# POSTECH-CVLab/RoDyGS

Measured on AMD Instinct MI355X. Metric: train-step fps at 1M dynamic Gaussians / 1080p (fwd+bwd+Adam, one camera per GPU per step), higher is better.
Workload: dtype f32; 1 GPU; 1000000 dynamic Gaussians + deformation MLP, 1920x1080, SH3, 100-frame synthetic video (BASELINE configs[2]); points=1000000, width=1920, height=1080, scene=uniform, frames=100, deferred_overflow_check=True, frame_order=orbit positions, bit-reversed, one_device=False, graph_replay=False, densify_stats=True, deterministic_backward=True, render_normal=True, parallelism=single GPU (frame-dp1), losses=photometric, sh_adam_in_backward=True, binning=bucket

## Files before the change

### rodygs_amd/csrc/rdg_common.h

```cpp
#pragma once
#include <hip/hip_runtime.h>
#include <stdint.h>
#include <stddef.h>
#include "../../include/rodygs_hip.h"

#define RDG_TILE 16
#define RDG_TILE_PIX 256
#define RDG_WAVE 64

#define RDG_NEAR_CULL 0.2f
#define RDG_FOV_CLAMP 1.3f
#define RDG_DILATION 0.3f
#define RDG_ALPHA_CAP 0.99f
#define RDG_ALPHA_MIN (1.0f / 255.0f)
#define RDG_T_STOP 0.0001f
#define RDG_LAMBDA_FLOOR 0.1f

struct __attribute__((aligned(64))) RdgRec {
    float4 q0, q1, q2, q3;
};

#define RDG_GROW 16

static inline size_t rdg_align_up(size_t x, size_t a) { return (x + a - 1) / a * a; }
// ... 230 lines not shown
                              const float* grow, float* posebuf, float* dmeans3D, float* dmeans2D, float* dshs,
                              float* dcolors, float* dopac, float* dscales, float* drots, float* dcov3D,
                              float* dview, hipStream_t s, const RdgShAdam* sh_adam = nullptr);

int rdg_launch_preprocess_fwd_views(const RdgDev& d, int32_t nviews, int32_t stride, int32_t row0,
                                    const float* means3D, const float* shs, const float* opac, const float* scales,
                                    const float* rots, const float* views, const float* proj, void* geom_ws,
                                    int32_t* radii, hipStream_t s);
int rdg_launch_preprocess_bwd_views(const RdgDev& d, int32_t nviews, int32_t stride, const float* means3D,
                                    const float* shs, const float* opac, const float* scales, const float* rots,
                                    const float* views, const float* proj, const int32_t* radii, const void* geom_ws,
                                    const float* grow, float* posebuf, float* dmeans3D, float* dmeans2D, float* dshs,
                                    float* dopac, float* dscales, float* drots, hipStream_t s);
int rdg_launch_pose_reduce_views(int nviews, int view_rows, int nblk, const float* views, float* posebuf, float* part,
                                 float* dviews, hipStream_t s);

#ifdef __HIPCC__
template <int CTRL, int ROW_MASK = 0xf, int BANK_MASK = 0xf, bool BOUND = true>
__device__ __forceinline__ float rdg_dpp(float x) {
    return __builtin_bit_cast(float, __builtin_amdgcn_update_dpp(0, __builtin_bit_cast(int, x), CTRL, ROW_MASK,
                                                                 BANK_MASK, BOUND));
}
template <int CTRL, int ROW_MASK = 0xf, int BANK_MASK = 0xf, bool BOUND = true>
__device__ __forceinline__ uint32_t rdg_dpp_u(uint32_t x) {
    return (uint32_t)__builtin_amdgcn_update_dpp(0, (int)x, CTRL, ROW_MASK, BANK_MASK, BOUND);
}
__device__ __forceinline__ float rdg_wave_sum_to63(float x) {
    x += rdg_dpp<0xB1>(x);
    x += rdg_dpp<0x4E>(x);
    x += rdg_dpp<0x141>(x);
    x += rdg_dpp<0x140>(x);
    x += rdg_dpp<0x142, 0xa>(x);
    x += rdg_dpp<0x143, 0xc>(x);
    return x;
}
__device__ __forceinline__ float rdg_wave_sum_all(float x) {
    x = rdg_wave_sum_to63(x);
    return __builtin_bit_cast(float, __builtin_amdgcn_readlane(__builtin_bit_cast(int, x), 63));
}
__device__ __forceinline__ void rdg_wave_lds_sync() {
    __builtin_amdgcn_fence(__ATOMIC_RELEASE, "wavefront");
    __builtin_amdgcn_wave_barrier();
    __builtin_amdgcn_fence(__ATOMIC_ACQUIRE, "wavefront");
}

template <bool NT = true>
__device__ __forceinline__ void rdg_rows_to_lds(const float* __restrict__ g, long long first_row, long long n_rows,
                                                int row, int stride, float* S, int lane) {
    const long long base = first_row * row, total = n_rows * row;
    const float inv_row = 1.0f / (float)row;
    if ((row & 3) == 0 && (((uintptr_t)g) & 15) == 0) {
        typedef float rdg_nt4 __attribute__((ext_vector_type(4)));
        for (int v0 = lane; v0 < 16 * row; v0 += 256) {
            rdg_nt4 val[4];
#pragma unroll
            for (int u = 0; u < 4; ++u) {
                const int v = v0 + 64 * u;
                const long long e = base + 4ll * v;
                if (v < 16 * row && e < total)
                    val[u] = NT ? __builtin_nontemporal_load(reinterpret_cast<const rdg_nt4*>(g + e))
                                : *reinterpret_cast<const rdg_nt4*>(g + e);
            }
#pragma unroll
            for (int u = 0; u < 4; ++u) {
                const int v = v0 + 64 * u;
                const long long e = base + 4ll * v;
                if (v < 16 * row && e < total) {
                    const int gi = (int)(((float)(4 * v) + 0.5f) * inv_row);
                    float* dst = S + gi * stride + (4 * v - gi * row);
                    dst[0] = val[u].x; dst[1] = val[u].y; dst[2] = val[u].z; dst[3] = val[u].w;
                }
            }
        }
    } else {
        for (int idx = lane; idx < 64 * row; idx += 64) {
            const long long e = base + idx;
            if (e < total) {
                const int gi = (int)(((float)idx + 0.5f) * inv_row);
                S[gi * stride + (idx - gi * row)] = g[e];
            }
        }
    }
}
__device__ __forceinline__ void rdg_lds_to_rows(float* __restrict__ g, long long first_row, long long n_rows, int row,
                                                int stride, const float* S, int lane) {
    const long long base = first_row * row, total = n_rows * row;
    const float inv_row = 1.0f / (float)row;
    if ((row & 3) == 0 && (((uintptr_t)g) & 15) == 0) {
        for (int v = lane; v < 16 * row; v += 64) {
            const long long e = base + 4ll * v;
            if (e < total) {
                const int gi = (int)(((float)(4 * v) + 0.5f) * inv_row);
                const float* src = S + gi * stride + (4 * v - gi * row);
                typedef float rdg_nt4 __attribute__((ext_vector_type(4)));
                const rdg_nt4 val = {src[0], src[1], src[2], src[3]};
                __builtin_nontemporal_store(val, reinterpret_cast<rdg_nt4*>(g + e));
            }
        }
    } else {
        for (int idx = lane; idx < 64 * row; idx += 64) {
            const long long e = base + idx;
            if (e < total) {
                const int gi = (int)(((float)idx + 0.5f) * inv_row);
                g[e] = S[gi * stride + (idx - gi * row)];
            }
        }
    }
}
template <bool ACC>
__device__ __forceinline__ void rdg_lds_acc_rows(float* __restrict__ g, long long first_row, long long n_rows, int row,
                                                 int stride, const float* S, int lane) {
    const long long base = first_row * row, total = n_rows * row;
    const float inv_row = 1.0f / (float)row;
    if ((row & 3) == 0 && (((uintptr_t)g) & 15) == 0) {
        for (int v = lane; v < 16 * row; v += 64) {
            const long long e = base + 4ll * v;
            if (e < total) {
                const int gi = (int)(((float)(4 * v) + 0.5f) * inv_row);
                const float* src = S + gi * stride + (4 * v - gi * row);
                float4* dst = reinterpret_cast<float4*>(g + e);
                float4 val = make_float4(src[0], src[1], src[2], src[3]);
                if (ACC) { const float4 o = *dst; val.x += o.x; val.y += o.y; val.z += o.z; val.w += o.w; }
                *dst = val;
            }
        }
    } else {
        for (int idx = lane; idx < 64 * row; idx += 64) {
            const long long e = base + idx;
            if (e < total) {
                const int gi = (int)(((float)idx + 0.5f) * inv_row);
                const float val = S[gi * stride + (idx - gi * row)];
                g[e] = ACC ? g[e] + val : val;
            }
        }
    }
}
__device__ __forceinline__ void rdg_adam_elem(float& p, float g, float& m, float& v, float st, float b1, float b2,
                                              float omb1, float omb2, float eps, float bc2_sqrt) {
    m = __fmaf_rn(b1, m, omb1 * g);
    v = __fmaf_rn(b2, v, (omb2 * g) * g);
    p = __fmaf_rn(-st, m / (sqrtf(v) / bc2_sqrt + eps), p);
}


#define RDG_FAC 20
__device__ __forceinline__ float rdg_fac_grad(const float* Frow, int idx) {
    const int k = (idx * 171) >> 9;
    return Frow[k] * Frow[16 + (idx - 3 * k)];
}
__device__ __forceinline__ void rdg_lds_adam_rows_fac(float* __restrict__ p, const RdgShAdam ad, long long first_row,
                                                      long long n_rows, int row, int stride, const float* S,
                                                      const float* F, int lane) {
    const long long base = first_row * row, total = n_rows * row;
    const float inv_row = 1.0f / (float)row;
    typedef float rdg_nt4 __attribute__((ext_vector_type(4)));
    if ((row & 3) == 0 && ((((uintptr_t)p) | ((uintptr_t)ad.m) | ((uintptr_t)ad.v)) & 15) == 0) {
#define RDG_ADAM_UNROLL 4
        for (int v0 = lane; v0 < 16 * row; v0 += 64 * RDG_ADAM_UNROLL) {
            rdg_nt4 mm[RDG_ADAM_UNROLL], vv[RDG_ADAM_UNROLL];
#pragma unroll
            for (int u = 0; u < RDG_ADAM_UNROLL; ++u) {
                const int v = v0 + 64 * u;
                const long long e = base + 4ll * v;
                if (v < 16 * row && e < total) {
                    mm[u] = __builtin_nontemporal_load(reinterpret_cast<const rdg_nt4*>(ad.m + e));
                    vv[u] = __builtin_nontemporal_load(reinterpret_cast<const rdg_nt4*>(ad.v + e));
// ... 90 lines not shown
```

### rodygs_amd/csrc/rdg_preprocess_fwd.hip

```cpp
#include "rdg_common.h"

#define SH_C0 0.28209479177387814f
#define SH_C1 0.4886025119029199f
__device__ static const float SH_C2[5] = {1.0925484305920792f, -1.0925484305920792f, 0.31539156525252005f,
                                          -1.0925484305920792f, 0.5462742152960396f};
__device__ static const float SH_C3[7] = {-0.5900435899266435f, 2.890611442640554f, -0.4570457994644658f,
                                          0.3731763325901154f,  -0.4570457994644658f, 1.445305721320277f,
                                          -0.5900435899266435f};

__device__ __forceinline__ void rdg_rect(float px, float py, int radius, int gx, int gy, int& x0, int& y0,
                                         int& x1, int& y1) {
    float r = (float)radius;
    x0 = min(gx, max(0, (int)((px - r) / (float)RDG_TILE)));
    y0 = min(gy, max(0, (int)((py - r) / (float)RDG_TILE)));
    x1 = min(gx, max(0, (int)((((px + r) + (float)RDG_TILE) - 1.0f) / (float)RDG_TILE)));
    y1 = min(gy, max(0, (int)((((py + r) + (float)RDG_TILE) - 1.0f) / (float)RDG_TILE)));
}

__device__ __forceinline__ float rdg_ln_exact_ops(float x) {
    const uint32_t u = __float_as_uint(x);
    int e = (int)(u >> 23) - 127;
    float m = __uint_as_float((u & 0x007fffffu) | 0x3f800000u);
    if (m > 1.41421354f) { m = m * 0.5f; e += 1; }
    const float s = (m - 1.0f) / (m + 1.0f);
    const float s2 = s * s;
    float p = 0.111111111f * s2 + 0.142857143f;
    p = p * s2 + 0.2f;
    p = p * s2 + 0.333333333f;
    p = p * s2 + 1.0f;
    return (2.0f * s) * p + (float)e * 0.693147181f;
}

__device__ __forceinline__ void rdg_splat_rect(const float4 q0, const float4 q1, const float inv_cyy, int gx, int gy, int cull,
                                               int& x0, int& y0, int& x1, int& y1) {
    rdg_rect(q0.x, q0.y, __float_as_int(q1.w), gx, gy, x0, y0, x1, y1);
    if (!cull) return;
    const float a = q0.z, b = q0.w, o = q1.y;
    const float t255 = 255.0f * o;
    if (!(t255 >= 0.99f)) { x1 = x0; y1 = y0; return; }
    const float r2 = (2.0f * (rdg_ln_exact_ops(t255) + 0.02f)) * 1.001f;
    const float cyy = 1.0f / inv_cyy;
    const float c_eff = (b * b) / a + inv_cyy;
    const float cxx = (c_eff * cyy) / a;
    const float hx = sqrtf(r2 * cxx), hy = sqrtf(r2 * cyy);
    const float lox = fmaxf(ceilf(q0.x - hx), 0.0f), hix = fminf(floorf(q0.x + hx), (float)(gx * RDG_TILE - 1));
    const float loy = fmaxf(ceilf(q0.y - hy), 0.0f), hiy = fminf(floorf(q0.y + hy), (float)(gy * RDG_TILE - 1));
    if (hix < lox || hiy < loy) { x1 = x0; y1 = y0; return; }
    x0 = max(x0, (int)lox >> 4); x1 = min(x1, ((int)hix >> 4) + 1);
    y0 = max(y0, (int)loy >> 4); y1 = min(y1, ((int)hiy >> 4) + 1);
    if (x1 < x0) x1 = x0;
    if (y1 < y0) y1 = y0;
}
__device__ __forceinline__ uint4 rdg_pack_rectd(int x0, int y0, int x1, int y1, float depth, uint32_t tiles) {
    if (tiles == 0u) return make_uint4(0u, 0u, 0u, 0u);
    return make_uint4((uint32_t)x0 | ((uint32_t)y0 << 16), (uint32_t)x1 | ((uint32_t)y1 << 16), __float_as_uint(depth), tiles);
}

template <bool MULTI>
__global__ void __launch_bounds__(RDG_PRE_BLOCK)
rdg_preprocess_fwd_kernel(RdgDev d, const float* __restrict__ view_b, const float* __restrict__ proj,
                          const float* __restrict__ means3D_b, const float* __restrict__ shs,
                          const float* __restrict__ colors, const float* __restrict__ opac,
                          const float* __restrict__ scales, const float* __restrict__ rots_b,
                          const float* __restrict__ cov3Dp, RdgRec* __restrict__ rec_b,
                          uint32_t* __restrict__ tiles_touched_b, uint8_t* __restrict__ clampedm_b,
                          uint32_t* __restrict__ block_sums_b, int32_t* __restrict__ radii_b, int nviews_arg,
                          int vstride_arg, int blk0_arg, uint4* __restrict__ rectd_b) {
    const int nviews = MULTI ? nviews_arg : 1, vstride = MULTI ? vstride_arg : 0;
    const int bid = (MULTI ? blk0_arg : 0) + (int)blockIdx.x;
    const int i = bid * RDG_PRE_BLOCK + threadIdx.x;
    __shared__ float sSH[RDG_PRE_BLOCK / 64][64 * 49];
    const int sh_row = d.M * 3, sh_stride = sh_row | 1;
    const long long wave_first = (long long)bid * RDG_PRE_BLOCK + (threadIdx.x >> 6) * 64;
    if (shs && wave_first < d.P) {
        rdg_rows_to_lds(shs, wave_first, d.P, sh_row, sh_stride, sSH[threadIdx.x >> 6], threadIdx.x & 63);
        rdg_wave_lds_sync();
    }
    __shared__ uint32_t wsum[RDG_PRE_BLOCK / RDG_WAVE];
    for (int vw = 0; vw < nviews; ++vw) {
    const size_t vo = (size_t)vw * vstride;
    const float* __restrict__ view = view_b + 16 * vw;
    const float* __restrict__ means3D = means3D_b + vo * 3;
    const float* __restrict__ rots = rots_b ? rots_b + vo * 4 : nullptr;
    RdgRec* __restrict__ rec = rec_b + vo;
    uint32_t* __restrict__ tiles_touched = tiles_touched_b + vo;
    uint8_t* __restrict__ clampedm = clampedm_b + vo;
    int32_t* __restrict__ radii = radii_b + vo;
    uint32_t* __restrict__ block_sums = block_sums_b + vo / RDG_PRE_BLOCK;
    uint4* __restrict__ rectd = rectd_b + vo;
    float V[16], Pm[16];
#pragma unroll
    for (int k = 0; k < 16; ++k) { V[k] = view[k]; Pm[k] = proj[k]; }
    uint32_t my_tiles = 0;
    if (i < d.P) {
        int radius_out = 0;
        uint8_t cl = 0;
        uint4 rd = make_uint4(0u, 0u, 0u, 0u);
        RdgRec R;
        R.q0 = make_float4(0.f, 0.f, 0.f, 0.f);
        R.q1 = R.q0; R.q2 = R.q0; R.q3 = R.q0;
        const float x = means3D[3 * i + 0], y = means3D[3 * i + 1], z = means3D[3 * i + 2];
        const float vx = ((V[0] * x + V[4] * y) + V[8] * z) + V[12];
        const float vy = ((V[1] * x + V[5] * y) + V[9] * z) + V[13];
        const float vz = ((V[2] * x + V[6] * y) + V[10] * z) + V[14];
        bool valid = vz > RDG_NEAR_CULL;
        if (valid) {
            const float hx = ((Pm[0] * vx + Pm[4] * vy) + Pm[8] * vz) + Pm[12];
            const float hy = ((Pm[1] * vx + Pm[5] * vy) + Pm[9] * vz) + Pm[13];
            const float hw = ((Pm[3] * vx + Pm[7] * vy) + Pm[11] * vz) + Pm[15];
            const float pw = 1.0f / (hw + 1e-7f);
            const float ndc_x = hx * pw, ndc_y = hy * pw;

            float S00, S01, S02, S11, S12, S22;
            float nx = 0.f, ny = 0.f, nz = 0.f;
            if (cov3Dp) {
                S00 = cov3Dp[6 * i + 0]; S01 = cov3Dp[6 * i + 1]; S02 = cov3Dp[6 * i + 2];
                S11 = cov3Dp[6 * i + 3]; S12 = cov3Dp[6 * i + 4]; S22 = cov3Dp[6 * i + 5];
            } else {
                const float s0 = d.smod * scales[3 * i + 0], s1 = d.smod * scales[3 * i + 1],
                            s2 = d.smod * scales[3 * i + 2];
                const float4 q = reinterpret_cast<const float4*>(rots)[i];
                const float r = q.x, qx = q.y, qy = q.z, qz = q.w;
                const float R00 = 1.0f - 2.0f * (qy * qy + qz * qz), R01 = 2.0f * (qx * qy - r * qz),
                            R02 = 2.0f * (qx * qz + r * qy);
                const float R10 = 2.0f * (qx * qy + r * qz), R11 = 1.0f - 2.0f * (qx * qx + qz * qz),
                            R12 = 2.0f * (qy * qz - r * qx);
                const float R20 = 2.0f * (qx * qz - r * qy), R21 = 2.0f * (qy * qz + r * qx),
                            R22 = 1.0f - 2.0f * (qx * qx + qy * qy);
                const float L00 = R00 * s0, L01 = R01 * s1, L02 = R02 * s2;
                const float L10 = R10 * s0, L11 = R11 * s1, L12 = R12 * s2;
                const float L20 = R20 * s0, L21 = R21 * s1, L22 = R22 * s2;
                S00 = (L00 * L00 + L01 * L01) + L02 * L02;
                S01 = (L00 * L10 + L01 * L11) + L02 * L12;
                S02 = (L00 * L20 + L01 * L21) + L02 * L22;
                S11 = (L10 * L10 + L11 * L11) + L12 * L12;
                S12 = (L10 * L20 + L11 * L21) + L12 * L22;
                S22 = (L20 * L20 + L21 * L21) + L22 * L22;
                if (d.render_normal) {
                    const float sc0 = scales[3 * i + 0], sc1 = scales[3 * i + 1], sc2 = scales[3 * i + 2];
                    int k = 0; float sm = sc0;
                    if (sc1 < sm) { sm = sc1; k = 1; }
                    if (sc2 < sm) { sm = sc2; k = 2; }
                    const float n0 = k == 0 ? R00 : (k == 1 ? R01 : R02);
                    const float n1 = k == 0 ? R10 : (k == 1 ? R11 : R12);
                    const float n2 = k == 0 ? R20 : (k == 1 ? R21 : R22);
                    float nvx = (V[0] * n0 + V[4] * n1) + V[8] * n2;
                    float nvy = (V[1] * n0 + V[5] * n1) + V[9] * n2;
                    float nvz = (V[2] * n0 + V[6] * n1) + V[10] * n2;
                    const float dotv = (nvx * vx + nvy * vy) + nvz * vz;
                    const float sg = dotv > 0.f ? -1.0f : 1.0f;
                    nx = nvx * sg; ny = nvy * sg; nz = nvz * sg;
                }
            }
            const float limx = RDG_FOV_CLAMP * d.tanx, limy = RDG_FOV_CLAMP * d.tany;
            const float txtz = vx / vz, tytz = vy / vz;
            const float tx = fminf(limx, fmaxf(-limx, txtz)) * vz;
            const float ty = fminf(limy, fmaxf(-limy, tytz)) * vz;
            const float J00 = d.fx / vz, J02 = -(d.fx * tx) / (vz * vz);
            const float J11 = d.fy / vz, J12 = -(d.fy * ty) / (vz * vz);
            const float T00 = J00 * V[0] + J02 * V[2], T01 = J00 * V[4] + J02 * V[6], T02 = J00 * V[8] + J02 * V[10];
            const float T10 = J11 * V[1] + J12 * V[2], T11 = J11 * V[5] + J12 * V[6], T12 = J11 * V[9] + J12 * V[10];
            const float u00 = (T00 * S00 + T01 * S01) + T02 * S02;
            const float u01 = (T00 * S01 + T01 * S11) + T02 * S12;
            const float u02 = (T00 * S02 + T01 * S12) + T02 * S22;
            const float u10 = (T10 * S00 + T11 * S01) + T12 * S02;
            const float u11 = (T10 * S01 + T11 * S11) + T12 * S12;
            const float u12 = (T10 * S02 + T11 * S12) + T12 * S22;
            const float ca = ((u00 * T00 + u01 * T01) + u02 * T02) + RDG_DILATION;
            const float cb = (u00 * T10 + u01 * T11) + u02 * T12;
            const float cc = ((u10 * T10 + u11 * T11) + u12 * T12) + RDG_DILATION;
            const float det = ca * cc - cb * cb;
            valid = det != 0.0f;
            if (valid) {
                const float det_inv = 1.0f / det;
                const float mid = 0.5f * (ca + cc);
                const float disc = sqrtf(fmaxf(RDG_LAMBDA_FLOOR, mid * mid - det));
                const float lam = fmaxf(mid + disc, mid - disc);
                const int radius = (int)ceilf(3.0f * sqrtf(lam));
                const float px = ((ndc_x + 1.0f) * (float)d.W - 1.0f) * 0.5f;
                const float py = ((ndc_y + 1.0f) * (float)d.H - 1.0f) * 0.5f;
                const float4 rq0 = make_float4(px, py, cc * det_inv, -cb * det_inv);
                const float4 rq1 = make_float4(ca * det_inv, opac[i], vz, __int_as_float(radius));
                const float inv_cyy = 1.0f / cc;
                int x0, y0, x1, y1;
                rdg_rect(px, py, radius, d.gx, d.gy, x0, y0, x1, y1);
                const int area = (x1 - x0) * (y1 - y0);
                if (area > 0) {
                    if (d.cull) rdg_splat_rect(rq0, rq1, inv_cyy, d.gx, d.gy, 1, x0, y0, x1, y1);
                    my_tiles = (uint32_t)((x1 - x0) * (y1 - y0));
                    rd = rdg_pack_rectd(x0, y0, x1, y1, vz, my_tiles);
                    radius_out = radius;
                    float cr, cg, cbl;
                    if (colors) {
                        cr = colors[3 * i + 0]; cg = colors[3 * i + 1]; cbl = colors[3 * i + 2];
                    } else {
                        const float camx = -((V[0] * V[12] + V[1] * V[13]) + V[2] * V[14]);
                        const float camy = -((V[4] * V[12] + V[5] * V[13]) + V[6] * V[14]);
                        const float camz = -((V[8] * V[12] + V[9] * V[13]) + V[10] * V[14]);
                        float dx = x - camx, dy = y - camy, dz = z - camz;
                        const float ln = sqrtf((dx * dx + dy * dy) + dz * dz);
                        dx = dx / ln; dy = dy / ln; dz = dz / ln;
                        const float* sh = sSH[threadIdx.x >> 6] + (threadIdx.x & 63) * sh_stride;
                        float res[3];
#pragma unroll
                        for (int c = 0; c < 3; ++c) res[c] = SH_C0 * sh[c];
                        if (d.deg > 0) {
#pragma unroll
                            for (int c = 0; c < 3; ++c)
                                res[c] = res[c] - SH_C1 * dy * sh[3 + c] + SH_C1 * dz * sh[6 + c] -
                                         SH_C1 * dx * sh[9 + c];
                            if (d.deg > 1) {
                                const float xx = dx * dx, yy = dy * dy, zz = dz * dz;
                                const float xy = dx * dy, yz = dy * dz, xz = dx * dz;
#pragma unroll
                                for (int c = 0; c < 3; ++c)
                                    res[c] = res[c] + SH_C2[0] * xy * sh[12 + c] + SH_C2[1] * yz * sh[15 + c] +
                                             SH_C2[2] * (2.0f * zz - xx - yy) * sh[18 + c] +
                                             SH_C2[3] * xz * sh[21 + c] + SH_C2[4] * (xx - yy) * sh[24 + c];
                                if (d.deg > 2) {
#pragma unroll
                                    for (int c = 0; c < 3; ++c)
                                        res[c] = res[c] + SH_C3[0] * dy * (3.0f * xx - yy) * sh[27 + c] +
                                                 SH_C3[1] * xy * dz * sh[30 + c] +
                                                 SH_C3[2] * dy * (4.0f * zz - xx - yy) * sh[33 + c] +
                                                 SH_C3[3] * dz * (2.0f * zz - 3.0f * xx - 3.0f * yy) * sh[36 + c] +
                                                 SH_C3[4] * dx * (4.0f * zz - xx - yy) * sh[39 + c] +
                                                 SH_C3[5] * dz * (xx - yy) * sh[42 + c] +
                                                 SH_C3[6] * dx * (xx - 3.0f * yy) * sh[45 + c];
                                }
                            }
                        }
                        res[0] += 0.5f; res[1] += 0.5f; res[2] += 0.5f;
                        if (res[0] < 0.f) cl |= 1;
                        if (res[1] < 0.f) cl |= 2;
                        if (res[2] < 0.f) cl |= 4;
                        cr = fmaxf(res[0], 0.f); cg = fmaxf(res[1], 0.f); cbl = fmaxf(res[2], 0.f);
                    }
                    R.q0 = rq0;
                    R.q1 = rq1;
                    R.q2 = make_float4(cr, cg, cbl, inv_cyy);
                    R.q3 = make_float4(nx, ny, nz, 0.f);
                }
            }
        }
        rec[i] = R;
        tiles_touched[i] = my_tiles;
        rectd[i] = rd;
        clampedm[i] = cl;
        radii[i] = radius_out;
    }
    uint32_t inc = rdg_wave_scan_incl(my_tiles);
    const uint32_t lane = threadIdx.x & 63, w = threadIdx.x >> 6;
    if (lane == 63) wsum[w] = inc;
    __syncthreads();
    if (threadIdx.x == 0) block_sums[bid] = wsum[0] + wsum[1] + wsum[2] + wsum[3];
    if (nviews > 1) __syncthreads();
    }
}

__global__ void __launch_bounds__(1024) rdg_scan_block_sums_kernel(uint32_t* __restrict__ block_sums, int nblk,
                                                                   int32_t* __restrict__ num_rendered,
                                                                   uint32_t* __restrict__ zero_buf, int zero_words,
                                                                   int32_t* __restrict__ nren_max) {
    for (int i = threadIdx.x; i < zero_words; i += 1024) zero_buf[i] = 0u;
    __shared__ uint32_t wtot[16];
    __shared__ unsigned long long wtot64[16];
    const uint32_t lane = threadIdx.x & 63, w = threadIdx.x >> 6;
    const int per = (nblk + 1023) / 1024;
    const int t0 = min(nblk, (int)threadIdx.x * per), t1 = min(nblk, t0 + per);
    uint32_t mine = 0;
    unsigned long long mine64 = 0ull;
    for (int c0 = t0; c0 < t1; c0 += 8) {
        uint32_t vv[8];
#pragma unroll
        for (int q = 0; q < 8; ++q) vv[q] = c0 + q < t1 ? block_sums[c0 + q] : 0u;
#pragma unroll
        for (int q = 0; q < 8; ++q) { mine += vv[q]; mine64 += vv[q]; }
// ... 112 lines not shown
```

### rodygs_amd/csrc/rdg_render.hip

```cpp
#include "rdg_common.h"

#define RDG_BATCH 256

__device__ __forceinline__ int rdg_tile_of_block(int bid, int n_tiles) {
    const int per = (n_tiles + 7) >> 3;
    return (bid & 7) * per + (bid >> 3);
}

__device__ __forceinline__ float rdg_edge_min(float a, float b2, float c, float inv_c, float ue, float v0, float v1) {
    const float t = b2 * ue;
    const float vs = __builtin_amdgcn_fmed3f(-0.5f * t * inv_c, v0, v1);
    return fmaf(fmaf(c, vs, t), vs, a * ue * ue);
}
__device__ __forceinline__ uint32_t rdg_quadrant_bits(const float4 q0, const float4 q1, const float inv_cyy, float X0, float Y0) {
    const float a = q0.z, b = q0.w, o = q1.y;
    const float c = (b * b) / a + inv_cyy;
    const float t255 = 255.0f * o;
    if (!(t255 >= 0.99f)) return 0u;
    const float det = a * c - b * b;
    if (!(det > 0.0f) || !(a > 0.0f) || !(c > 0.0f)) return 0u;
    const float r2 = 2.0f * (__logf(t255) + 0.02f) * 1.001f;
    const float inv_a = 1.0f / a, inv_c = 1.0f / c, b2 = 2.0f * b;
    uint32_t bits = 0u;
#pragma unroll
    for (int qy = 0; qy < 2; ++qy) {
        const float v1 = q0.y - (Y0 + 8.0f * qy), v0 = v1 - 7.0f;
#pragma unroll
        for (int qx = 0; qx < 2; ++qx) {
            const float u1 = q0.x - (X0 + 8.0f * qx), u0 = u1 - 7.0f;
            const bool inside = u0 <= 0.0f && u1 >= 0.0f && v0 <= 0.0f && v1 >= 0.0f;
            const float m = fminf(fminf(rdg_edge_min(a, b2, c, inv_c, u0, v0, v1), rdg_edge_min(a, b2, c, inv_c, u1, v0, v1)),
                                  fminf(rdg_edge_min(c, b2, a, inv_a, v0, u0, u1), rdg_edge_min(c, b2, a, inv_a, v1, u0, u1)));
            bits |= (uint32_t)(inside || !(m > r2)) << (qy * 2 + qx);
        }
    }
    return bits;
}

#define RDG_NEG_LOG2E (-1.4426950408889634f)
struct RdgConicS { float hA, beta, gam; };
__device__ __forceinline__ RdgConicS rdg_stage_conic(float a, float b, float inv_cyy) {
    const float A2 = RDG_NEG_LOG2E * a, B = RDG_NEG_LOG2E * b;
    RdgConicS s;
    s.hA = 0.5f * A2;
    s.beta = (A2 < 0.0f) ? B / A2 : 0.0f;
    s.gam = (0.5f * RDG_NEG_LOG2E) * inv_cyy;
    return s;
}
__device__ __forceinline__ float rdg_log2_gauss(float hA, float beta, float gam, float dx, float dy) {
    const float w = fmaf(beta, dy, dx);
    return fmaf(hA * w, w, (gam * dy) * dy);
}
__device__ __forceinline__ float rdg_log2_gauss_w(float hA, float beta, float gam, float dx, float dy, float& w) {
    w = fmaf(beta, dy, dx);
    return fmaf(hA * w, w, (gam * dy) * dy);
}

__device__ __forceinline__ bool rdg_any(bool p) { return __builtin_amdgcn_ballot_w64(p) != 0ull; }
__device__ __forceinline__ bool rdg_all(bool p) { return __builtin_amdgcn_ballot_w64(!p) == 0ull; }

__device__ __forceinline__ unsigned long long rdg_uniform_u64(unsigned long long v) {
    const uint32_t lo = __builtin_amdgcn_readfirstlane((uint32_t)v);
    const uint32_t hi = __builtin_amdgcn_readfirstlane((uint32_t)(v >> 32));
    return ((unsigned long long)hi << 32) | lo;
}

#define RDG_THR_LIVE (0x80000000u | 0x3b808081u)
#define RDG_THR_DONE 0xffffffffu
template <bool NORMAL, bool CAPPED>
__device__ __forceinline__ void rdg_fwd_walk(unsigned long long mask, const unsigned long long cap, const int sbase,
                                             const uint32_t wbase, const char* sQ0, const char* sQ1, const char* sQ2,
                                             const char* sQ3, const float pixx, const float pixy,
                                             unsigned long long& seen, uint32_t& thrU, float& T,
                                             uint32_t& last_contributor, float& C0, float& C1, float& C2, float& Dp,
                                             float& N0, float& N1, float& N2) {
    while (mask) {
        const int jb = __builtin_ctzll(mask);
        asm("s_bitset0_b64 %0, %1" : "+s"(mask) : "s"(jb));
        int aj = (jb << 4) + sbase;
        asm volatile("" : "+v"(aj));
#ifdef RDG_ABL_FXSALU
        asm volatile("s_add_u32 s90, s90, 1\n\ts_add_u32 s91, s91, 1\n\ts_add_u32 s90, s90, 1\n\ts_add_u32 s91, s91, 1\n\t"
                     "s_add_u32 s90, s90, 1\n\ts_add_u32 s91, s91, 1\n\ts_add_u32 s90, s90, 1\n\ts_add_u32 s91, s91, 1" ::: "s90", "s91", "scc");
#endif
#ifdef RDG_ABL_FXVALU
        { float xa = T, xb = C0;
          asm volatile("v_mov_b32 %0, %1\n\tv_mov_b32 %1, %0\n\tv_mov_b32 %0, %1\n\tv_mov_b32 %1, %0\n\t"
                       "v_mov_b32 %0, %1\n\tv_mov_b32 %1, %0\n\tv_mov_b32 %0, %1\n\tv_mov_b32 %1, %0" : "+v"(xa), "+v"(xb)); }
#endif
        const float4 q0 = *(const float4*)(sQ0 + aj);
        const float2 q1 = *(const float2*)(sQ1 + aj);
        const float dx = q0.x - pixx, dy = q0.y - pixy;
        const float power = rdg_log2_gauss(q0.z, q0.w, q1.x, dx, dy);
        float alpha = q1.y * __builtin_amdgcn_exp2f(power);
        if (CAPPED && ((cap >> jb) & 1ull)) {
            asm volatile("; opacity above the cap" ::: "memory");
            alpha = fminf(RDG_ALPHA_CAP, alpha);
        }
        const uint32_t key = (__float_as_uint(power) & 0x80000000u) | __float_as_uint(alpha);
        const unsigned long long cand = __builtin_amdgcn_ballot_w64(key >= thrU);
        if (!cand) continue;
        asm("s_bitset1_b64 %0, %1" : "+s"(seen) : "s"(jb));
        float aeff;
        asm("v_cndmask_b32_e64 %0, 0, %1, %2" : "=v"(aeff) : "v"(alpha), "s"(cand));
        float test_T = T * (1.0f - aeff);
        float wgt = aeff * T;
        const float4 q2 = *(const float4*)(sQ2 + aj);
        const uint32_t idx = wbase + (uint32_t)jb;
        unsigned long long upd = cand;
        const unsigned long long stopm = __builtin_amdgcn_ballot_w64(test_T < RDG_T_STOP);
        if (stopm) {
            const bool stop = test_T < RDG_T_STOP;
            upd &= ~stopm;
            wgt = stop ? 0.0f : wgt;
            test_T = stop ? T : test_T;
            thrU = stop ? RDG_THR_DONE : thrU;
            if (rdg_all(thrU == RDG_THR_DONE)) { mask = 0ull; }
        }
        T = test_T;
        asm volatile("s_mov_b64 exec, %1\n\tv_mov_b32 %0, %2\n\ts_mov_b64 exec, -1"
                     : "+v"(last_contributor) : "s"(upd), "s"(idx));
        C0 += wgt * q2.x; C1 += wgt * q2.y; C2 += wgt * q2.z;
        Dp += wgt * q2.w;
        if (NORMAL) {
            const float4 q3 = *(const float4*)(sQ3 + aj);
            N0 += wgt * q3.x; N1 += wgt * q3.y; N2 += wgt * q3.z;
        }
    }
}


template <bool NORMAL>
__device__ __forceinline__ void
rdg_fwd_composite(const int k_begin, const int k_end, const uint2 range, const float X0, const float Y0, const float pixx,
                  const float pixy, const uint32_t* __restrict__ point_list, const RdgRec* __restrict__ rec,
                  unsigned long long* __restrict__ hit, float4* sQ0, float4* sQ1, float4* sQ2, float4* sQ3,
                  unsigned long long (*sMask)[4], unsigned long long* sCap, uint32_t& thrU, float& T, float& C0, float& C1,
                  float& C2, float& Dp, float& N0, float& N1, float& N2, uint32_t& last_contributor) {
    const int tid = threadIdx.x;
    const int lane = tid & 63, wv = tid >> 6;
    const int rounds = (k_end - k_begin + RDG_BATCH - 1) / RDG_BATCH;
    for (int r = 0; r < rounds; ++r) {
        if (__syncthreads_count(thrU == RDG_THR_DONE) == 256) break;
        const int k = k_begin + r * RDG_BATCH + tid;
        uint32_t qbits = 0;
        bool over_cap = false;
        if (k < k_end) {
            const uint32_t id = point_list[range.x + k];
            const RdgRec* p = rec + id;
            const float4 q0 = p->q0, q1 = p->q1, q2 = p->q2;
            const RdgConicS cs = rdg_stage_conic(q0.z, q0.w, q2.w);
            sQ0[tid] = make_float4(q0.x, q0.y, cs.hA, cs.beta);
            *(float2*)&sQ1[tid] = make_float2(cs.gam, q1.y);
            sQ2[tid] = make_float4(q2.x, q2.y, q2.z, q1.z);
            if (NORMAL) sQ3[tid] = p->q3;
            qbits = rdg_quadrant_bits(q0, q1, q2.w, X0, Y0);
            over_cap = q1.y > RDG_ALPHA_CAP;
        }
#pragma unroll
        for (int q = 0; q < 4; ++q) {
            const unsigned long long m = __ballot((qbits >> q) & 1u);
            if (lane == 0) sMask[q][wv] = m;
        }
        {
            const unsigned long long m = __ballot(over_cap);
            if (lane == 0) sCap[wv] = m;
        }
        __syncthreads();
#pragma unroll 1
        for (int s = 0; s < 4; ++s) {
            if (rdg_all(thrU == RDG_THR_DONE)) break;
            const unsigned long long mask = rdg_uniform_u64(sMask[wv][s]);
            const unsigned long long cap = rdg_uniform_u64(sCap[s]);
            unsigned long long seen = 0ull;
            const uint32_t wbase = (uint32_t)(k_begin + r * RDG_BATCH + s * 64 + 1);
            if (cap)
                rdg_fwd_walk<NORMAL, true>(mask, cap, s * 1024, wbase, (const char*)sQ0, (const char*)sQ1, (const char*)sQ2,
                                           (const char*)sQ3, pixx, pixy, seen, thrU, T, last_contributor, C0, C1, C2, Dp,
                                           N0, N1, N2);
            else
                rdg_fwd_walk<NORMAL, false>(mask, cap, s * 1024, wbase, (const char*)sQ0, (const char*)sQ1, (const char*)sQ2,
                                            (const char*)sQ3, pixx, pixy, seen, thrU, T, last_contributor, C0, C1, C2, Dp,
                                            N0, N1, N2);
            if (lane == 0 && seen) hit[(size_t)((k_begin >> 6) + r * 4 + s) * 4 + wv] = seen;
        }
    }
}

template <bool NORMAL>
__global__ void __launch_bounds__(256)
rdg_render_fwd_kernel(int W, int H, int gx, int n_tiles, const float* __restrict__ bg,
                      const uint2* __restrict__ ranges, const uint32_t* __restrict__ point_list,
                      const RdgRec* __restrict__ rec, long long capacity, const int32_t* __restrict__ num_rendered,
                      float* __restrict__ final_T, uint32_t* __restrict__ n_contrib, float* __restrict__ out_color,
                      float* __restrict__ out_depth, float* __restrict__ out_normal, float* __restrict__ out_alpha,
                      unsigned long long* __restrict__ hitbits, int split_min, uint4* __restrict__ zero_buf,
                      long long zero_n16) {
    if (zero_buf) {
        const long long per = (zero_n16 + gridDim.x - 1) / gridDim.x;
        const long long z0 = per * blockIdx.x, z1 = z0 + per < zero_n16 ? z0 + per : zero_n16;
        for (long long i = z0 + threadIdx.x; i < z1; i += 256) zero_buf[i] = make_uint4(0u, 0u, 0u, 0u);
    }
    const int tile = rdg_tile_of_block(blockIdx.x, n_tiles);
    if (tile >= n_tiles) return;
    __shared__ float4 sQ0[RDG_BATCH], sQ1[RDG_BATCH], sQ2[RDG_BATCH], sQ3[RDG_BATCH];
    __shared__ unsigned long long sMask[4][4];
    __shared__ unsigned long long sCap[4];
#ifdef RDG_ABL_FPAD
    __shared__ float sPad[RDG_ABL_FPAD];
// ... 268 lines not shown
        } else {
            hipLaunchKernelGGL(rdg_render_seg_kernel<false>, dim3(gseg), dim3(256), 0, s, d.W, d.H, d.gx, ranges, plist, rec,
                               sp_header, sp_work, seg_pix, hitbits);
            hipLaunchKernelGGL(rdg_render_seg_combine_kernel<false>, dim3(gtile), dim3(256), 0, s, d.W, d.H, d.gx, bg,
                               sp_header, sp_tiles, (const float*)seg_pix, final_T, n_contrib, out_color, out_depth,
                               out_normal, out_alpha);
        }
    }
    return rdg_check_hip(hipGetLastError(), "render_fwd launch");
}

#ifndef RDG_RING
#define RDG_RING 4
#endif
#define RDG_RING_Q 6
template <bool HAS_DEPTH, bool DET>
__device__ __forceinline__ void rdg_ring_flush(float (*ring)[16][RDG_RING_Q], int n, int lane, float scale, int foff,
                                               float* __restrict__ grow) {
    __builtin_amdgcn_fence(__ATOMIC_RELEASE, "wavefront");
    __builtin_amdgcn_wave_barrier();
    __builtin_amdgcn_fence(__ATOMIC_ACQUIRE, "wavefront");
    const int c = lane & 15;
    for (int e0 = 0; e0 < n; e0 += 4) {
        const int e = e0 + (lane >> 4);
        if (e < n && c < (HAS_DEPTH ? 10 : 9)) {
            const float* r = &ring[e][0][0] + foff;
            constexpr int G = 2 * RDG_RING_Q;
            const float v = (((r[0] + r[G]) + (r[2 * G] + r[3 * G])) + ((r[4 * G] + r[5 * G]) + (r[6 * G] + r[7 * G]))) * scale;
#ifdef RDG_ABL_NOATOMIC
            if (v == 123.456f) atomicAdd(grow + (size_t)__float_as_uint(ring[e][1][4]) * RDG_GROW + c, v);
#else
            if (DET) grow[(size_t)__float_as_uint(ring[e][1][4]) * (4 * RDG_GROW) + c] = v;
            else if (v != 0.0f) atomicAdd(grow + (size_t)__float_as_uint(ring[e][1][4]) * RDG_GROW + c, v);
#endif
        }
    }
    __builtin_amdgcn_fence(__ATOMIC_RELEASE, "wavefront");
    __builtin_amdgcn_wave_barrier();
    __builtin_amdgcn_fence(__ATOMIC_ACQUIRE, "wavefront");
}

template <bool HAS_DEPTH, bool CAPPED, bool DET, bool ALLBELOW, bool HAS_NORMAL>
__device__ __forceinline__ void rdg_bwd_walk(unsigned long long mask, const unsigned long long cap, const int sbase,
                                             const char* sQ0, const char* sQ1, const char* sQ2, const char* sQ3,
                                             const float pixx, const float pixy, const int jthr, const float dLp0,
                                             const float dLp1, const float dLp2, const float dLd, const float dLn0,
                                             const float dLn1, const float dLn2, const int lane,
                                             float (*ring)[16][RDG_RING_Q], const float flush_scale, const int flush_off,
                                             float* __restrict__ grow, float& T, float& behind, int& ring_n) {
    while (mask) {
        const int jb = __builtin_ctzll(mask);
        asm("s_bitset0_b64 %0, %1" : "+s"(mask) : "s"(jb));
        int aj = (jb << 4) + sbase;
        asm volatile("" : "+v"(aj));
        const float4 q0 = *(const float4*)(sQ0 + aj);
        const float4 q1 = *(const float4*)(sQ1 + aj);
        const float dx = q0.x - pixx, dy = q0.y - pixy;
        float wsk;
        const float power = rdg_log2_gauss_w(q0.z, q0.w, q1.x, dx, dy, wsk);
        const float G = __builtin_amdgcn_exp2f(power);
        float alpha = q1.y * G;
        const bool capped = CAPPED && ((cap >> jb) & 1ull);
        if (capped) {
            asm volatile("; opacity above the cap" ::: "memory");
            alpha = fminf(RDG_ALPHA_CAP, alpha);
        }
        const uint32_t key = (__float_as_uint(power) & 0x80000000u) | __float_as_uint(alpha);
        const bool hit = ALLBELOW ? key >= RDG_THR_LIVE : ((jb > jthr) && key >= RDG_THR_LIVE);
        if (!rdg_any(hit)) continue;
#ifdef RDG_ABL_PREONLY
        if (G != 123.456f) continue;
#endif
        const float4 q2 = *(const float4*)(sQ2 + aj);
        const float Gm = hit ? G : 0.0f;
        float aeff = q1.y * Gm;
        if (capped) {
            asm volatile("; opacity above the cap" ::: "memory");
            aeff = fminf(RDG_ALPHA_CAP, aeff);
        }
        const float inv1ma = __builtin_amdgcn_rcpf(1.0f - aeff);
        T = T * inv1ma;
        const float dch = aeff * T;
        float s_ = q2.x * dLp0 + q2.y * dLp1 + q2.z * dLp2;
        if (HAS_DEPTH) s_ += q1.z * dLd;
        if (HAS_NORMAL) {
            const float4 q3 = *(const float4*)(sQ3 + aj);
            s_ += q3.x * dLn0 + q3.y * dLn1 + q3.z * dLn2;
        }
        const float e_ = s_ - behind;
        behind = fmaf(aeff, e_, behind);
        const float dL_dalpha = e_ * T;
        const float t0 = Gm * dL_dalpha;
        const float t1 = t0 * wsk;
        const float t2 = t1 * wsk;
        const float c0 = dch * dLp0, c1 = dch * dLp1, c2 = dch * dLp2, cd = HAS_DEPTH ? dch * dLd : 0.0f;
        float r0, r1, r2, r3 = 0.0f;
#ifdef RDG_ABL_NODPP
        r0 = t0 + t1; r1 = t2 + c0; r2 = c1 + c2; r3 = cd;
        if (true) {
        } else if (HAS_DEPTH) {
#else
        if (HAS_DEPTH) {
#endif
            asm volatile(
                "s_nop 1\n\t"
                "v_add_f32_dpp %[r0], %[t0], %[t0] row_half_mirror row_mask:0xf bank_mask:0x5\n\t"
                "v_add_f32_dpp %[r0], %[t1], %[t1] row_half_mirror row_mask:0xf bank_mask:0xa\n\t"
                "v_add_f32_dpp %[r1], %[t2], %[t2] row_half_mirror row_mask:0xf bank_mask:0x5\n\t"
                "v_add_f32_dpp %[r1], %[c0], %[c0] row_half_mirror row_mask:0xf bank_mask:0xa\n\t"
                "v_add_f32_dpp %[r2], %[c1], %[c1] row_half_mirror row_mask:0xf bank_mask:0x5\n\t"
                "v_add_f32_dpp %[r2], %[c2], %[c2] row_half_mirror row_mask:0xf bank_mask:0xa\n\t"
                "v_add_f32_dpp %[r3], %[cd], %[cd] row_half_mirror row_mask:0xf bank_mask:0xf\n\t"
                "v_add_f32_dpp %[r0], %[r0], %[r0] quad_perm:[1,0,3,2] row_mask:0xf bank_mask:0xf\n\t"
                "v_add_f32_dpp %[r1], %[r1], %[r1] quad_perm:[1,0,3,2] row_mask:0xf bank_mask:0xf\n\t"
                "v_add_f32_dpp %[r2], %[r2], %[r2] quad_perm:[1,0,3,2] row_mask:0xf bank_mask:0xf\n\t"
                "v_add_f32_dpp %[r3], %[r3], %[r3] quad_perm:[1,0,3,2] row_mask:0xf bank_mask:0xf\n\t"
                "v_add_f32_dpp %[r0], %[r0], %[r0] quad_perm:[2,3,0,1] row_mask:0xf bank_mask:0xf\n\t"
                "v_add_f32_dpp %[r1], %[r1], %[r1] quad_perm:[2,3,0,1] row_mask:0xf bank_mask:0xf\n\t"
                "v_add_f32_dpp %[r2], %[r2], %[r2] quad_perm:[2,3,0,1] row_mask:0xf bank_mask:0xf\n\t"
                "v_add_f32_dpp %[r3], %[r3], %[r3] quad_perm:[2,3,0,1] row_mask:0xf bank_mask:0xf"
                : [r0] "=&v"(r0), [r1] "=&v"(r1), [r2] "=&v"(r2), [r3] "=&v"(r3)
                : [t0] "v"(t0), [t1] "v"(t1), [t2] "v"(t2), [c0] "v"(c0), [c1] "v"(c1), [c2] "v"(c2), [cd] "v"(cd));
        } else {
            asm volatile(
                "s_nop 1\n\t"
                "v_add_f32_dpp %[r0], %[t0], %[t0] row_half_mirror row_mask:0xf bank_mask:0x5\n\t"
                "v_add_f32_dpp %[r0], %[t1], %[t1] row_half_mirror row_mask:0xf bank_mask:0xa\n\t"
                "v_add_f32_dpp %[r1], %[t2], %[t2] row_half_mirror row_mask:0xf bank_mask:0x5\n\t"
                "v_add_f32_dpp %[r1], %[c0], %[c0] row_half_mirror row_mask:0xf bank_mask:0xa\n\t"
                "v_add_f32_dpp %[r2], %[c1], %[c1] row_half_mirror row_mask:0xf bank_mask:0x5\n\t"
                "v_add_f32_dpp %[r2], %[c2], %[c2] row_half_mirror row_mask:0xf bank_mask:0xa\n\t"
                "v_add_f32_dpp %[r0], %[r0], %[r0] quad_perm:[1,0,3,2] row_mask:0xf bank_mask:0xf\n\t"
                "v_add_f32_dpp %[r1], %[r1], %[r1] quad_perm:[1,0,3,2] row_mask:0xf bank_mask:0xf\n\t"
                "v_add_f32_dpp %[r2], %[r2], %[r2] quad_perm:[1,0,3,2] row_mask:0xf bank_mask:0xf\n\t"
                "v_add_f32_dpp %[r0], %[r0], %[r0] quad_perm:[2,3,0,1] row_mask:0xf bank_mask:0xf\n\t"
                "v_add_f32_dpp %[r1], %[r1], %[r1] quad_perm:[2,3,0,1] row_mask:0xf bank_mask:0xf\n\t"
                "v_add_f32_dpp %[r2], %[r2], %[r2] quad_perm:[2,3,0,1] row_mask:0xf bank_mask:0xf"
                : [r0] "=&v"(r0), [r1] "=&v"(r1), [r2] "=&v"(r2)
                : [t0] "v"(t0), [t1] "v"(t1), [t2] "v"(t2), [c0] "v"(c0), [c1] "v"(c1), [c2] "v"(c2));
        }
        const float m1 = r0 * dy;
        const float m2 = m1 * dy;
        {
#if defined(RDG_PARK_ALL)
            {
                float* gr = &ring[ring_n][lane >> 2][0];
                gr[0] = r0; gr[1] = r1; gr[2] = r2; gr[3] = m1; gr[4] = ((lane >> 2) == 1) ? q2.w : m2;
                if (HAS_DEPTH) gr[5] = r3;
            }
#else
#ifdef RDG_ABL_NOPARK
            if (lane == 63 && m2 == 123.456f) {
#else
            if ((lane & 3) == 0) {
#endif
                float* gr = &ring[ring_n][lane >> 2][0];
                gr[0] = r0; gr[1] = r1; gr[2] = r2; gr[3] = m1; gr[4] = m2;
                if (HAS_DEPTH) gr[5] = r3;
                if (lane == 4) gr[4] = q2.w;
            }
#endif
            if (++ring_n == RDG_RING) {
                rdg_ring_flush<HAS_DEPTH, DET>(ring, ring_n, lane, flush_scale, flush_off, grow);
                ring_n = 0;
            }
        }
    }
}

template <bool HAS_DEPTH, bool DET, bool HAS_NORMAL>
// ... 263 lines not shown
```

Before: 724.2 frames/s.

## Prefetch per-Gaussian inputs and SH rows into registers before LDS staging

The preprocess kernel now issues the SH-row loads into registers and also loads scales, opacity, means, rotations, cov3D and colors up front, before committing the SH rows to LDS. The point is to overlap global-memory latency of the per-Gaussian attributes with the SH staging, instead of loading them serially after the sync. Empty asm barriers pin the prefetched values in VGPRs. Separately, the render kernels add keep-alive asm on the .w lane of float4 LDS reads so they stay as full 128-bit loads. The cost is higher register pressure, which could lower occupancy.

```diff
diff --git a/rodygs_amd/csrc/rdg_common.h b/rodygs_amd/csrc/rdg_common.h
--- a/rodygs_amd/csrc/rdg_common.h
+++ b/rodygs_amd/csrc/rdg_common.h
@@ -336,6 +336,38 @@
         }
     }
 }
+#define RDG_ROWS_REGS 12
+typedef float rdg_f4v __attribute__((ext_vector_type(4)));
+template <bool NT = true>
+__device__ __forceinline__ bool rdg_rows_issue(const float* __restrict__ g, long long first_row, long long n_rows, int row,
+                                               int lane, rdg_f4v (&val)[RDG_ROWS_REGS]) {
+    if ((row & 3) != 0 || row > 4 * RDG_ROWS_REGS || (((uintptr_t)g) & 15) != 0) return false;
+    const long long base = first_row * row, total = n_rows * row;
+#pragma unroll
+    for (int u = 0; u < RDG_ROWS_REGS; ++u) {
+        if (4 * u < row) {
+            long long e = base + 4ll * (lane + 64 * u);
+            e = e < total ? e : total - 4;
+            val[u] = NT ? __builtin_nontemporal_load(reinterpret_cast<const rdg_f4v*>(g + e))
+                        : *reinterpret_cast<const rdg_f4v*>(g + e);
+        }
+    }
+    return true;
+}
+__device__ __forceinline__ void rdg_rows_commit(long long first_row, long long n_rows, int row, int stride, float* S,
+                                                int lane, const rdg_f4v (&val)[RDG_ROWS_REGS]) {
+    const long long base = first_row * row, total = n_rows * row;
+    const float inv_row = 1.0f / (float)row;
+#pragma unroll
+    for (int u = 0; u < RDG_ROWS_REGS; ++u) {
+        const int v = lane + 64 * u;
+        if (4 * u < row && base + 4ll * v < total) {
+            const int gi = (int)(((float)(4 * v) + 0.5f) * inv_row);
+            float* dst = S + gi * stride + (4 * v - gi * row);
+            dst[0] = val[u].x; dst[1] = val[u].y; dst[2] = val[u].z; dst[3] = val[u].w;
+        }
+    }
+}
 __device__ __forceinline__ void rdg_lds_to_rows(float* __restrict__ g, long long first_row, long long n_rows, int row,
                                                 int stride, const float* S, int lane) {
     const long long base = first_row * row, total = n_rows * row;
diff --git a/rodygs_amd/csrc/rdg_preprocess_fwd.hip b/rodygs_amd/csrc/rdg_preprocess_fwd.hip
--- a/rodygs_amd/csrc/rdg_preprocess_fwd.hip
+++ b/rodygs_amd/csrc/rdg_preprocess_fwd.hip
@@ -72,8 +72,38 @@
     __shared__ float sSH[RDG_PRE_BLOCK / 64][64 * 49];
     const int sh_row = d.M * 3, sh_stride = sh_row | 1;
     const long long wave_first = (long long)bid * RDG_PRE_BLOCK + (threadIdx.x >> 6) * 64;
-    if (shs && wave_first < d.P) {
-        rdg_rows_to_lds(shs, wave_first, d.P, sh_row, sh_stride, sSH[threadIdx.x >> 6], threadIdx.x & 63);
+    const bool stage_sh = shs && wave_first < d.P;
+    rdg_f4v shv[RDG_ROWS_REGS];
+    bool sh_in_regs = false;
+    if (stage_sh) sh_in_regs = rdg_rows_issue(shs, wave_first, d.P, sh_row, threadIdx.x & 63, shv);
+    const int ic = min(i, d.P - 1);
+    const float* __restrict__ scales_v = scales ? scales : means3D_b;
+    const float* __restrict__ rots_v = rots_b ? rots_b : cov3Dp;
+    float sc0 = scales_v[3 * ic + 0], sc1 = scales_v[3 * ic + 1], sc2 = scales_v[3 * ic + 2];
+    float op = opac[ic];
+    float x = 0.f, y = 0.f, z = 0.f;
+    float4 q = make_float4(0.f, 0.f, 0.f, 0.f);
+    float V[16], Pm[16];
+#pragma unroll
+    for (int k = 0; k < 16; ++k) Pm[k] = proj[k];
+    if (!MULTI) {
+        x = means3D_b[3 * ic + 0]; y = means3D_b[3 * ic + 1]; z = means3D_b[3 * ic + 2];
+        q = reinterpret_cast<const float4*>(rots_v)[ic];
+#pragma unroll
+        for (int k = 0; k < 16; ++k) V[k] = view_b[k];
+    }
+    float cv[6] = {0.f, 0.f, 0.f, 0.f, 0.f, 0.f}, col[3] = {0.f, 0.f, 0.f};
+    if (cov3Dp) {
+#pragma unroll
+        for (int k = 0; k < 6; ++k) cv[k] = cov3Dp[6 * ic + k];
+    }
+    if (colors) {
+#pragma unroll
+        for (int k = 0; k < 3; ++k) col[k] = colors[3 * ic + k];
+    }
+    if (stage_sh) {
+        if (sh_in_regs) rdg_rows_commit(wave_first, d.P, sh_row, sh_stride, sSH[threadIdx.x >> 6], threadIdx.x & 63, shv);
+        else rdg_rows_to_lds(shs, wave_first, d.P, sh_row, sh_stride, sSH[threadIdx.x >> 6], threadIdx.x & 63);
         rdg_wave_lds_sync();
     }
     __shared__ uint32_t wsum[RDG_PRE_BLOCK / RDG_WAVE];
@@ -81,16 +111,22 @@
     const size_t vo = (size_t)vw * vstride;
     const float* __restrict__ view = view_b + 16 * vw;
     const float* __restrict__ means3D = means3D_b + vo * 3;
-    const float* __restrict__ rots = rots_b ? rots_b + vo * 4 : nullptr;
+    if (MULTI) {
+        x = means3D[3 * ic + 0]; y = means3D[3 * ic + 1]; z = means3D[3 * ic + 2];
+        q = reinterpret_cast<const float4*>(rots_v + vo * 4)[ic];
+#pragma unroll
+        for (int k = 0; k < 16; ++k) V[k] = view[k];
+    }
+    asm volatile("" : "+v"(x), "+v"(y), "+v"(z), "+v"(q.x), "+v"(q.y), "+v"(q.z), "+v"(q.w), "+v"(sc0), "+v"(sc1), "+v"(sc2),
+                 "+v"(op));
+    asm volatile("" : "+v"(cv[0]), "+v"(cv[1]), "+v"(cv[2]), "+v"(cv[3]), "+v"(cv[4]), "+v"(cv[5]), "+v"(col[0]), "+v"(col[1]),
+                 "+v"(col[2]));
     RdgRec* __restrict__ rec = rec_b + vo;
     uint32_t* __restrict__ tiles_touched = tiles_touched_b + vo;
     uint8_t* __restrict__ clampedm = clampedm_b + vo;
     int32_t* __restrict__ radii = radii_b + vo;
     uint32_t* __restrict__ block_sums = block_sums_b + vo / RDG_PRE_BLOCK;
     uint4* __restrict__ rectd = rectd_b + vo;
-    float V[16], Pm[16];
-#pragma unroll
-    for (int k = 0; k < 16; ++k) { V[k] = view[k]; Pm[k] = proj[k]; }
     uint32_t my_tiles = 0;
     if (i < d.P) {
         int radius_out = 0;
@@ -99,7 +135,6 @@
         RdgRec R;
         R.q0 = make_float4(0.f, 0.f, 0.f, 0.f);
         R.q1 = R.q0; R.q2 = R.q0; R.q3 = R.q0;
-        const float x = means3D[3 * i + 0], y = means3D[3 * i + 1], z = means3D[3 * i + 2];
         const float vx = ((V[0] * x + V[4] * y) + V[8] * z) + V[12];
         const float vy = ((V[1] * x + V[5] * y) + V[9] * z) + V[13];
         const float vz = ((V[2] * x + V[6] * y) + V[10] * z) + V[14];
@@ -114,12 +149,10 @@
             float S00, S01, S02, S11, S12, S22;
             float nx = 0.f, ny = 0.f, nz = 0.f;
             if (cov3Dp) {
-                S00 = cov3Dp[6 * i + 0]; S01 = cov3Dp[6 * i + 1]; S02 = cov3Dp[6 * i + 2];
-                S11 = cov3Dp[6 * i + 3]; S12 = cov3Dp[6 * i + 4]; S22 = cov3Dp[6 * i + 5];
+                S00 = cv[0]; S01 = cv[1]; S02 = cv[2];
+                S11 = cv[3]; S12 = cv[4]; S22 = cv[5];
             } else {
-                const float s0 = d.smod * scales[3 * i + 0], s1 = d.smod * scales[3 * i + 1],
-                            s2 = d.smod * scales[3 * i + 2];
-                const float4 q = reinterpret_cast<const float4*>(rots)[i];
+                const float s0 = d.smod * sc0, s1 = d.smod * sc1, s2 = d.smod * sc2;
                 const float r = q.x, qx = q.y, qy = q.z, qz = q.w;
                 const float R00 = 1.0f - 2.0f * (qy * qy + qz * qz), R01 = 2.0f * (qx * qy - r * qz),
                             R02 = 2.0f * (qx * qz + r * qy);
@@ -137,7 +170,6 @@
                 S12 = (L10 * L20 + L11 * L21) + L12 * L22;
                 S22 = (L20 * L20 + L21 * L21) + L22 * L22;
                 if (d.render_normal) {
-                    const float sc0 = scales[3 * i + 0], sc1 = scales[3 * i + 1], sc2 = scales[3 * i + 2];
                     int k = 0; float sm = sc0;
                     if (sc1 < sm) { sm = sc1; k = 1; }
                     if (sc2 < sm) { sm = sc2; k = 2; }
@@ -180,7 +212,7 @@
                 const float px = ((ndc_x + 1.0f) * (float)d.W - 1.0f) * 0.5f;
                 const float py = ((ndc_y + 1.0f) * (float)d.H - 1.0f) * 0.5f;
                 const float4 rq0 = make_float4(px, py, cc * det_inv, -cb * det_inv);
-                const float4 rq1 = make_float4(ca * det_inv, opac[i], vz, __int_as_float(radius));
+                const float4 rq1 = make_float4(ca * det_inv, op, vz, __int_as_float(radius));
                 const float inv_cyy = 1.0f / cc;
                 int x0, y0, x1, y1;
                 rdg_rect(px, py, radius, d.gx, d.gy, x0, y0, x1, y1);
@@ -192,7 +224,7 @@
                     radius_out = radius;
                     float cr, cg, cbl;
                     if (colors) {
-                        cr = colors[3 * i + 0]; cg = colors[3 * i + 1]; cbl = colors[3 * i + 2];
+                        cr = col[0]; cg = col[1]; cbl = col[2];
                     } else {
                         const float camx = -((V[0] * V[12] + V[1] * V[13]) + V[2] * V[14]);
                         const float camy = -((V[4] * V[12] + V[5] * V[13]) + V[6] * V[14]);
diff --git a/rodygs_amd/csrc/rdg_render.hip b/rodygs_amd/csrc/rdg_render.hip
--- a/rodygs_amd/csrc/rdg_render.hip
+++ b/rodygs_amd/csrc/rdg_render.hip
@@ -65,6 +65,7 @@
     return ((unsigned long long)hi << 32) | lo;
 }
 
+__device__ __forceinline__ void rdg_keep_w(const float4& q) { asm volatile("" :: "v"(q.w)); }
 #define RDG_THR_LIVE (0x80000000u | 0x3b808081u)
 #define RDG_THR_DONE 0xffffffffu
 template <bool NORMAL, bool CAPPED>
@@ -125,6 +126,7 @@
         if (NORMAL) {
             const float4 q3 = *(const float4*)(sQ3 + aj);
             N0 += wgt * q3.x; N1 += wgt * q3.y; N2 += wgt * q3.z;
+            rdg_keep_w(q3);
         }
     }
 }
@@ -559,10 +561,11 @@
         T = T * inv1ma;
         const float dch = aeff * T;
         float s_ = q2.x * dLp0 + q2.y * dLp1 + q2.z * dLp2;
-        if (HAS_DEPTH) s_ += q1.z * dLd;
+        if (HAS_DEPTH) { s_ += q1.z * dLd; rdg_keep_w(q1); }
         if (HAS_NORMAL) {
             const float4 q3 = *(const float4*)(sQ3 + aj);
             s_ += q3.x * dLn0 + q3.y * dLn1 + q3.z * dLn2;
+            rdg_keep_w(q3);
         }
         const float e_ = s_ - behind;
         behind = fmaf(aeff, e_, behind);
```

Result: faster. 733.9 frames/s, median of 5 (+1.3%).
